# nv-tlabs/ASE

Hardware: NVIDIA H100
Metric: training env-steps/sec HumanoidAMPGetup 4096 envs/GPU (higher is better)
Workload: dtype f32 (3xFP16 scaled hi/lo tensor-core products, fp32 accumulate)

## Files before the change

ase_b200/csrc/gemm_tc.cu:

```cuda
#include <cuda.h>
#include <cuda_fp16.h>
#include <vector>
#include <unordered_map>
#include <string.h>
#include <stdlib.h>
#include "common.cuh"
#include "kernels.h"
#include "tc_common.cuh"

namespace ase {


template <bool H>
__device__ __forceinline__ void epilogue_rows(const TcEpi& e, const float* cs, int cs_ld, float* s_colsum, int row0, int nrows, int BNT, int m0, int n0, int lane) {
  const bool vec_ok = ((e.ldc & 3) == 0) && ((reinterpret_cast<uintptr_t>(e.C) & 15) == 0) &&
                      (!e.mask_mode || e.mask_bits || (((e.ldm & 3) == 0) && ((reinterpret_cast<uintptr_t>(e.mask_src) & 15) == 0)));
  const bool add_bias = e.bias && (!e.accumulate || blockIdx.z == 0);
  const uintptr_t pal = H ? 7 : 15;
  const bool pvec = e.Chi && ((e.ldp & 3) == 0) && ((reinterpret_cast<uintptr_t>(e.Chi) & pal) == 0) && ((reinterpret_cast<uintptr_t>(e.Clo) & pal) == 0);
  const float cscale = (H && e.Chi && e.c_scale) ? *e.c_scale : 1.0f;
  const bool use_bits = e.mask_mode == 1 && e.mask_bits != nullptr;
  const int nib_shift = 4 * (lane & 7);
  float amax = 0.0f;
#pragma unroll 1
  for (int cc = lane * 4; cc < ((BNT + 127) & ~127); cc += 128) {
    const int n = n0 + cc;
    const int rem = (cc < BNT) ? e.N - n : 0;
    const bool full = rem >= 4;
    const int nvalid = full ? 4 : (rem > 0 ? rem : 0);
    float bv[4] = {0.0f, 0.0f, 0.0f, 0.0f};
    if (add_bias) for (int j = 0; j < nvalid; ++j) bv[j] = e.bias[n + j];
    float cs4[4] = {0.0f, 0.0f, 0.0f, 0.0f};
#pragma unroll 4
    for (int r = 0; r < nrows; ++r) {
      const int row = row0 + r, m = m0 + row;
      if (m >= e.M) break;
      const float4 t = (cc < BNT) ? lds128(cs + row * cs_ld + cc) : make_float4(0.0f, 0.0f, 0.0f, 0.0f);
      float x[4] = {t.x + bv[0], t.y + bv[1], t.z + bv[2], t.w + bv[3]};
      float* cp = e.C + (int64_t)m * e.ldc + n;
      if (e.accumulate) {
        if (vec_ok && full) asm volatile("red.global.add.v4.f32 [%0], {%1, %2, %3, %4};" ::"l"(cp), "f"(x[0]), "f"(x[1]), "f"(x[2]), "f"(x[3]) : "memory");
        else for (int j = 0; j < nvalid; ++j) atomicAdd(cp + j, x[j]);
        continue;
      }
      if (e.act == 1) { for (int j = 0; j < 4; ++j) x[j] = fmaxf(x[j], 0.0f); }
      else if (e.act == 2) { for (int j = 0; j < 4; ++j) x[j] = tanhf(x[j]); }
      if (e.relu_bits) {
        uint32_t w = 0;
#pragma unroll
        for (int j = 0; j < 4; ++j) w |= (j < nvalid && x[j] > 0.0f) ? (1u << j) : 0u;
        w <<= nib_shift;
        w |= __shfl_xor_sync(0xffffffffu, w, 1); w |= __shfl_xor_sync(0xffffffffu, w, 2); w |= __shfl_xor_sync(0xffffffffu, w, 4);
        if ((lane & 7) == 0 && nvalid > 0) e.relu_bits[(int64_t)m * e.ldrb + (n >> 5)] = w;
      }
      if (use_bits) {
        const uint32_t w = (nvalid > 0 && !(e.debug & 16)) ? e.mask_bits[(int64_t)m * e.ldmb + (n >> 5)] >> nib_shift : 0xFu;
#pragma unroll
        for (int j = 0; j < 4; ++j) x[j] = ((w >> j) & 1u) ? x[j] : 0.0f;
      } else if (e.mask_mode && !(e.debug & 16) && nvalid > 0) {
        const float* mp = e.mask_src + (int64_t)m * e.ldm + n;
        float mv[4] = {0.0f, 0.0f, 0.0f, 0.0f};
        if (vec_ok && full) { const float4 q = *reinterpret_cast<const float4*>(mp); mv[0] = q.x; mv[1] = q.y; mv[2] = q.z; mv[3] = q.w; }
        else for (int j = 0; j < nvalid; ++j) mv[j] = mp[j];
        if (e.mask_mode == 1) { for (int j = 0; j < 4; ++j) x[j] = (mv[j] > 0.0f) ? x[j] : 0.0f; }
        else { for (int j = 0; j < 4; ++j) x[j] *= (1.0f - mv[j] * mv[j]); }
      }
      if (e.skip_c || (e.debug & 128)) {}
      else if (vec_ok && full) *reinterpret_cast<float4*>(cp) = make_float4(x[0], x[1], x[2], x[3]);
      else for (int j = 0; j < nvalid; ++j) cp[j] = x[j];
#pragma unroll
      for (int j = 0; j < 4; ++j) { cs4[j] += x[j]; if (j < nvalid) amax = fmaxf(amax, fabsf(x[j])); }
      if (e.Chi && !(e.debug & 32) && nvalid > 0) {
        if (!H) {
          float h[4], l[4];
#pragma unroll
          for (int j = 0; j < 4; ++j) split_tf32(x[j], h[j], l[j]);
          float* hp = (float*)e.Chi + (int64_t)m * e.ldp + n; float* lp = (float*)e.Clo + (int64_t)m * e.ldp + n;
          if (pvec && full) { *reinterpret_cast<float4*>(hp) = make_float4(h[0], h[1], h[2], h[3]); *reinterpret_cast<float4*>(lp) = make_float4(l[0], l[1], l[2], l[3]); }
          else for (int j = 0; j < nvalid; ++j) { hp[j] = h[j]; lp[j] = l[j]; }
        } else {
          uint2 hv, lv;
          split_f16x2(x[0] * cscale, x[1] * cscale, hv.x, lv.x); split_f16x2(x[2] * cscale, x[3] * cscale, hv.y, lv.y);
          __half* hp = (__half*)e.Chi + (int64_t)m * e.ldp + n; __half* lp = (__half*)e.Clo + (int64_t)m * e.ldp + n;
          if (pvec && full) { *reinterpret_cast<uint2*>(hp) = hv; *reinterpret_cast<uint2*>(lp) = lv; }
          else {
            const uint32_t hw[2] = {hv.x, hv.y}, lw[2] = {lv.x, lv.y};
            for (int j = 0; j < nvalid; ++j) {
              hp[j] = __ushort_as_half((unsigned short)(hw[j >> 1] >> (16 * (j & 1))));
              lp[j] = __ushort_as_half((unsigned short)(lw[j >> 1] >> (16 * (j & 1))));
            }
          }
        }
      }
    }
    if (e.colsum && !e.accumulate && !(e.debug & 64)) for (int j = 0; j < nvalid; ++j) atomicAdd(s_colsum + cc + j, cs4[j]);
  }
  if ((e.c_amax || (H && e.Chi && e.flag)) && !e.accumulate) report_scale_miss(amax, cscale, e.c_amax, (H && e.Chi) ? e.flag : nullptr);
}

__device__ __forceinline__ bool epilogue_frag_ok(const TcEpi& e, int m0, int n0, int bm, int bn, bool H) {
  if (e.accumulate || m0 + bm > e.M || n0 + bn > e.N) return false;
  if ((e.ldc & 3) || (reinterpret_cast<uintptr_t>(e.C) & 15)) return false;
  if (e.bias && (reinterpret_cast<uintptr_t>(e.bias) & 15)) return false;
  if (e.Chi && (!H || (e.ldp & 7) || (reinterpret_cast<uintptr_t>(e.Chi) & 15) || (reinterpret_cast<uintptr_t>(e.Clo) & 15))) return false;
  if (e.mask_mode && !(e.mask_mode == 1 && e.mask_bits) && ((e.ldm & 3) || (reinterpret_cast<uintptr_t>(e.mask_src) & 15))) return false;
  return true;
}

template <class T, int N> struct FragArr {
  T v[N];
  __device__ __forceinline__ T& operator[](int i) { return v[i]; }
  __device__ __forceinline__ const T& operator[](int i) const { return v[i]; }
};

template <bool H, int NH>
__device__ __forceinline__ void epilogue_frag(const TcEpi& e, float (&acc)[NH][64], float* s_colsum, int m0, int n0, int wg, int t) {
  constexpr int NROW = 2 * NH;
  constexpr unsigned FULL = 0xffffffffu;
  const int lane = t & 31, q = lane & 3;
  const bool odd = q & 1;
  const int cq = ((q & 1) << 3) | ((q & 2) << 1);
  const int64_t m = m0 + wg * NH * 64 + 16 * (t >> 5) + (lane >> 2);
  const int n = n0 + cq;
  const float s1 = (H && e.a_inv) ? *e.a_inv : 1.0f;
  const float s2 = e.alpha * ((H && e.b_inv) ? *e.b_inv : 1.0f);
  const float cscale = (H && e.Chi && e.c_scale) ? *e.c_scale : 1.0f;
  const bool use_bits = e.mask_mode == 1 && e.mask_bits != nullptr;
  const uint32_t* mb = use_bits ? e.mask_bits + m * e.ldmb + (n0 >> 5) : nullptr;
  float* cp = e.C + m * e.ldc + n;
  __half* hp = (H && e.Chi) ? (__half*)e.Chi + m * e.ldp + n : nullptr;
  __half* lp = (H && e.Chi) ? (__half*)e.Clo + m * e.ldp + n : nullptr;
  const float* mp = (e.mask_mode && !use_bits) ? e.mask_src + m * e.ldm + n : nullptr;
  const float* bp = e.bias ? e.bias + n : nullptr;
  FragArr<uint32_t, NROW> mw, mwn;
#pragma unroll
  for (int k = 0; k < NROW; ++k) { mw[k] = 0; mwn[k] = 0; }
  if (use_bits) {
#pragma unroll
    for (int k = 0; k < NROW; ++k) mw[k] = __ldg(mb + (64 * (k >> 1) + 8 * (k & 1)) * e.ldmb);
  }
  float amax = 0.0f;
  FragArr<uint32_t, NROW> rbw;
#pragma unroll
  for (int k = 0; k < NROW; ++k) rbw[k] = 0;
#pragma unroll 1
  for (int g = 0; g < 8; ++g) {
    const int w = g >> 1;
    if (use_bits && !(g & 1) && w < 3) {
#pragma unroll
      for (int k = 0; k < NROW; ++k) mwn[k] = __ldg(mb + (64 * (k >> 1) + 8 * (k & 1)) * e.ldmb + w + 1);
    }
    const int c = 16 * g, sh = 16 * (g & 1) + cq;
    FragArr<float, 4> bv = {{0.0f, 0.0f, 0.0f, 0.0f}};
    if (bp) { const float4 b4 = *reinterpret_cast<const float4*>(bp + c); bv[0] = b4.x; bv[1] = b4.y; bv[2] = b4.z; bv[3] = b4.w; }
    FragArr<float, 4> csum = {{0.0f, 0.0f, 0.0f, 0.0f}};
#pragma unroll
    for (int k = 0; k < NROW; ++k) {
      const int64_t ro = 64 * (k >> 1) + 8 * (k & 1);
      const float* a = acc[k >> 1] + 2 * (k & 1);
      const float r0 = __shfl_xor_sync(FULL, odd ? a[0] : a[4], 1), r1 = __shfl_xor_sync(FULL, odd ? a[1] : a[5], 1);
      FragArr<float, 4> x;
      x[0] = odd ? r0 : a[0]; x[1] = odd ? r1 : a[1]; x[2] = odd ? a[4] : r0; x[3] = odd ? a[5] : r1;
#pragma unroll
      for (int j = 0; j < 4; ++j) x[j] = __fadd_rn(__fmul_rn(s2, __fmul_rn(s1, x[j])), bv[j]);
      if (e.act == 1) {
#pragma unroll
        for (int j = 0; j < 4; ++j) x[j] = fmaxf(x[j], 0.0f);
      } else if (e.act == 2) {
#pragma unroll
        for (int j = 0; j < 4; ++j) x[j] = tanhf(x[j]);
      }
      if (e.relu_bits) {
        uint32_t nib = 0;
#pragma unroll
        for (int j = 0; j < 4; ++j) nib |= (x[j] > 0.0f) ? (1u << j) : 0u;
        rbw[k] |= nib << sh;
      }
      if (use_bits) {
#pragma unroll
        for (int j = 0; j < 4; ++j) x[j] = ((mw[k] >> (sh + j)) & 1u) ? x[j] : 0.0f;
      } else if (mp) {
        const float4 q4 = *reinterpret_cast<const float4*>(mp + ro * e.ldm + c);
        const FragArr<float, 4> mv = {{q4.x, q4.y, q4.z, q4.w}};
        if (e.mask_mode == 1) {
#pragma unroll
          for (int j = 0; j < 4; ++j) x[j] = (mv[j] > 0.0f) ? x[j] : 0.0f;
        } else {
#pragma unroll
          for (int j = 0; j < 4; ++j) x[j] *= (1.0f - mv[j] * mv[j]);
        }
      }
      if (!e.skip_c) *reinterpret_cast<float4*>(cp + ro * e.ldc + c) = make_float4(x[0], x[1], x[2], x[3]);
#pragma unroll
      for (int j = 0; j < 4; ++j) { csum[j] += x[j]; amax = fmaxf(amax, fabsf(x[j])); }
      if (H && hp) {
        uint2 hv, lv;
        split_f16x2(x[0] * cscale, x[1] * cscale, hv.x, lv.x); split_f16x2(x[2] * cscale, x[3] * cscale, hv.y, lv.y);
        *reinterpret_cast<uint2*>(hp + ro * e.ldp + c) = hv;
        *reinterpret_cast<uint2*>(lp + ro * e.ldp + c) = lv;
      }
    }
    if (e.colsum) {
#pragma unroll
      for (int j = 0; j < 4; ++j) {
        float v = csum[j];
        v += __shfl_xor_sync(FULL, v, 4); v += __shfl_xor_sync(FULL, v, 8); v += __shfl_xor_sync(FULL, v, 16);
        if (lane < 4) atomicAdd(s_colsum + c + cq + j, v);
      }
    }
    if (e.relu_bits && (g & 1)) {
      uint32_t word = 0;
#pragma unroll
      for (int k = 0; k < NROW; ++k) {
        uint32_t v = rbw[k];
        v |= __shfl_xor_sync(FULL, v, 1); v |= __shfl_xor_sync(FULL, v, 2);
        if (q == k) word = v;
        rbw[k] = 0;
      }
      if (q < NROW) e.relu_bits[(m + 64 * (q >> 1) + 8 * (q & 1)) * e.ldrb + (n0 >> 5) + w] = word;
    }
    if (g & 1) {
#pragma unroll
      for (int k = 0; k < NROW; ++k) mw[k] = mwn[k];
    }
#pragma unroll
    for (int h = 0; h < NH; ++h)
#pragma unroll
      for (int i = 0; i < 56; ++i) acc[h][i] = acc[h][i + 8];
  }
  if (e.c_amax || (H && e.Chi && e.flag)) report_scale_miss(amax, cscale, e.c_amax, (H && e.Chi) ? e.flag : nullptr);
}

template <int BM, int BN> constexpr int tc_stages() { return (200 * 1024) / (256 * (BM + BN)); }

template <int BM, int BN, int STAGES>
struct TcSmem {
  static constexpr int A_BYTES = BM * 128;
  static constexpr int B_BYTES = BN * 128;
  static constexpr int STAGE_BYTES = 2 * A_BYTES + 2 * B_BYTES;
  static constexpr int COLSUM_OFF = STAGES * STAGE_BYTES + 256;
  static constexpr int TOTAL = COLSUM_OFF + 512 + 1024 ;
  static_assert(BM * (BN + 4) * 4 <= STAGES * STAGE_BYTES, "the generic store phase's staging tile lives over the ring");
};

template <int BN, bool AMN, bool BMN, bool H>
__device__ __forceinline__ void wg_mma(float (&d)[BN / 2], uint32_t a, uint32_t b, int k, int sd) {
  const uint64_t da = tc_desc<AMN>(a, k), db = tc_desc<BMN>(b, k);
  if constexpr (H) {
    if constexpr (BN == 128) wg_f16_n128<AMN, BMN>(d, da, db, sd); else wg_f16_n64<AMN, BMN>(d, da, db, sd);
  } else {
    if constexpr (BN == 128) wg_tf32_n128(d, da, db, sd); else wg_tf32_n64(d, da, db, sd);
  }
}

template <int BM, int BN, int STAGES, bool AMN, bool BMN, bool H>
__global__ void __launch_bounds__(TC_THREADS, 1)
gemm_tc_kernel(const __grid_constant__ CUtensorMap tmAhi, const __grid_constant__ CUtensorMap tmAlo,
               const __grid_constant__ CUtensorMap tmBhi, const __grid_constant__ CUtensorMap tmBlo, const TcEpi e) {
  static_assert(H || (!AMN && !BMN), "TF32 wgmma reads K-major operands only");
  static_assert(BM == 128 || BM == 256, "tile height");
  using SM = TcSmem<BM, BN, STAGES>;
  using F = TcFmt<H>;
  constexpr int R = BN / 2;
  constexpr int NH = BM / 128;
  extern __shared__ uint8_t smem_raw[];
  uint8_t* smem = reinterpret_cast<uint8_t*>((reinterpret_cast<uintptr_t>(smem_raw) + 1023) & ~uintptr_t(1023));
  uint64_t* full = reinterpret_cast<uint64_t*>(smem + STAGES * SM::STAGE_BYTES);
  uint64_t* empty = full + STAGES;

  const int warp = threadIdx.x >> 5, lane = threadIdx.x & 31;
  const int m0 = blockIdx.y * BM, n0 = blockIdx.x * BN;
  const int kb_begin = blockIdx.z * e.kb_per_split;
  const int nkb = min(e.kb_per_split, e.kb_total - kb_begin);

  if (threadIdx.x == 0) {
    asm volatile("prefetch.tensormap [%0];" ::"l"(reinterpret_cast<uint64_t>(&tmAhi)) : "memory");
    asm volatile("prefetch.tensormap [%0];" ::"l"(reinterpret_cast<uint64_t>(&tmAlo)) : "memory");
    asm volatile("prefetch.tensormap [%0];" ::"l"(reinterpret_cast<uint64_t>(&tmBhi)) : "memory");
    asm volatile("prefetch.tensormap [%0];" ::"l"(reinterpret_cast<uint64_t>(&tmBlo)) : "memory");
    for (int s = 0; s < STAGES; ++s) { mbar_init(&full[s], 1); mbar_init(&empty[s], 2); }
    asm volatile("fence.mbarrier_init.release.cluster;" ::: "memory");
  }
  float* s_colsum = reinterpret_cast<float*>(smem + SM::COLSUM_OFF);
  if (threadIdx.x < BN) s_colsum[threadIdx.x] = 0.0f;
  __syncthreads();
  pdl_sync();

  if (warp < 4) {
    asm volatile("setmaxnreg.dec.sync.aligned.u32 40;");
    if (warp == 0 && lane == 0) {
      for (int kb = 0; kb < nkb; ++kb) {
        const int s = kb % STAGES;
        const uint32_t ph = (kb / STAGES) & 1;
        mbar_wait(&empty[s], ph ^ 1);
        mbar_expect_tx(&full[s], SM::STAGE_BYTES);
        uint8_t* st = smem + s * SM::STAGE_BYTES;
        const int k0 = (kb_begin + kb) * F::BK;
        if (!AMN) {
          tma_load_2d(st, &tmAhi, &full[s], k0, m0);
          tma_load_2d(st + SM::A_BYTES, &tmAlo, &full[s], k0, m0);
        } else {
#pragma unroll
          for (int b = 0; b < BM / F::MN_BOX; ++b) {
            tma_load_2d(st + b * F::MN_BOX_BYTES, &tmAhi, &full[s], m0 + b * F::MN_BOX, k0);
            tma_load_2d(st + SM::A_BYTES + b * F::MN_BOX_BYTES, &tmAlo, &full[s], m0 + b * F::MN_BOX, k0);
          }
        }
        if (!BMN) {
          tma_load_2d(st + 2 * SM::A_BYTES, &tmBhi, &full[s], k0, n0);
          tma_load_2d(st + 2 * SM::A_BYTES + SM::B_BYTES, &tmBlo, &full[s], k0, n0);
        } else {
#pragma unroll
          for (int b = 0; b < BN / F::MN_BOX; ++b) {
            tma_load_2d(st + 2 * SM::A_BYTES + b * F::MN_BOX_BYTES, &tmBhi, &full[s], n0 + b * F::MN_BOX, k0);
            tma_load_2d(st + 2 * SM::A_BYTES + SM::B_BYTES + b * F::MN_BOX_BYTES, &tmBlo, &full[s], n0 + b * F::MN_BOX, k0);
          }
        }
      }
    }
    return;
  }
  asm volatile("setmaxnreg.inc.sync.aligned.u32 232;");
  const int wg = (warp >> 2) - 1;
  const int t = threadIdx.x & 127;
  const bool corrections = !(e.debug & 4);
  float acc[NH][R], part[R];
#pragma unroll
  for (int h = 0; h < NH; ++h)
#pragma unroll
    for (int j = 0; j < R; ++j) acc[h][j] = 0.0f;
  for (int kb = 0; kb < nkb; ++kb) {
    const int s = kb % STAGES;
    mbar_wait(&full[s], (kb / STAGES) & 1);
    const uint32_t sa = smem_u32(smem + s * SM::STAGE_BYTES);
    const uint32_t b_hi = sa + 2 * SM::A_BYTES, b_lo = b_hi + SM::B_BYTES;
#pragma unroll
    for (int h = 0; h < NH; ++h) {
      const uint32_t a_hi = sa + (wg * NH + h) * TC_M64_BYTES, a_lo = a_hi + SM::A_BYTES;
      wg_fence();
      if (corrections) {
#pragma unroll
        for (int k = 0; k < 4; ++k) {
          wg_mma<BN, AMN, BMN, H>(part, a_lo, b_hi, k, k > 0 ? 1 : 0);
          wg_mma<BN, AMN, BMN, H>(part, a_hi, b_lo, k, 1);
        }
      }
#pragma unroll
      for (int k = 0; k < 4; ++k) wg_mma<BN, AMN, BMN, H>(part, a_hi, b_hi, k, (corrections || k > 0) ? 1 : 0);
      wg_commit();
      wg_wait<0>();
      if (h == NH - 1 && t == 0) mbar_arrive(&empty[s]);
#pragma unroll
      for (int j = 0; j < R; ++j) acc[h][j] += part[j];
    }
  }
  const int et = threadIdx.x - 128;
  bool frag = false;
  if constexpr (BN == 128) frag = epilogue_frag_ok(e, m0, n0, BM, BN, H) && !(e.debug & 256);
  if (frag) {
    if constexpr (BN == 128) { if (!(e.debug & 1)) epilogue_frag<H, NH>(e, acc, s_colsum, m0, n0, wg, t); }
  } else {
    asm volatile("bar.sync 1, 256;" ::: "memory");
    float* cs = reinterpret_cast<float*>(smem);
    constexpr int CS_LD = BN + 4;
    const float s1 = (H && e.a_inv) ? *e.a_inv : 1.0f;
    const float s2 = e.alpha * ((H && e.b_inv) ? *e.b_inv : 1.0f);
#pragma unroll
    for (int h = 0; h < NH; ++h) {
      const int row = (wg * NH + h) * 64 + 16 * (t >> 5) + ((t & 31) >> 2);
      float* c0 = cs + row * CS_LD + 2 * (t & 3);
#pragma unroll
      for (int j = 0; j < R / 4; ++j) {
        const float* a = acc[h] + 4 * j;
        asm volatile("st.shared.v2.f32 [%0], {%1, %2};" ::"r"(smem_u32(c0 + 8 * j)), "f"(s2 * (s1 * a[0])), "f"(s2 * (s1 * a[1])) : "memory");
        asm volatile("st.shared.v2.f32 [%0], {%1, %2};" ::"r"(smem_u32(c0 + 8 * CS_LD + 8 * j)), "f"(s2 * (s1 * a[2])), "f"(s2 * (s1 * a[3])) : "memory");
      }
    }
    asm volatile("bar.sync 1, 256;" ::: "memory");
    constexpr int NRW = BM / 8;
    if (!(e.debug & 1)) epilogue_rows<H>(e, cs, CS_LD, s_colsum, (warp - 4) * NRW, NRW, BN, m0, n0, lane);
  }
  if (e.colsum && !e.accumulate) {
    asm volatile("bar.sync 1, 256;" ::: "memory");
    if (et < BN && n0 + et < e.N) atomicAdd(e.colsum + n0 + et, s_colsum[et]);
  }
}


__global__ void __launch_bounds__(256)
tc_prep_kernel(const float* __restrict__ src, int64_t ld, int rows, int cols, int rows_p, int cols_p, float* __restrict__ hi,
               float* __restrict__ lo) {
  const int64_t total = (int64_t)rows_p * cols_p;
  for (int64_t i = (int64_t)blockIdx.x * blockDim.x + threadIdx.x; i < total; i += (int64_t)gridDim.x * blockDim.x) {
    const int r = (int)(i / cols_p), c = (int)(i - (int64_t)r * cols_p);
    float h = 0.0f, l = 0.0f;
    if (r < rows && c < cols) split_tf32(src[(int64_t)r * ld + c], h, l);
    hi[i] = h; lo[i] = l;
  }
}

__global__ void __launch_bounds__(256)
tc_prep_t_kernel(const float* __restrict__ src, int64_t ld, int rows, int cols, int cols_p, float* __restrict__ hi,
                 float* __restrict__ lo) {
  __shared__ float tile[32][33];
  const int r0 = blockIdx.x * 32, c0 = blockIdx.y * 32, tx = threadIdx.x;
  for (int j = threadIdx.y; j < 32; j += 8) {
    const int c = c0 + j, r = r0 + tx;
    tile[j][tx] = (r < rows && c < cols) ? src[(int64_t)c * ld + r] : 0.0f;
  }
  __syncthreads();
  for (int j = threadIdx.y; j < 32; j += 8) {
    const int64_t o = (int64_t)(r0 + j) * cols_p + c0 + tx;
    float h, l;
    split_tf32(tile[tx][j], h, l);
    hi[o] = h; lo[o] = l;
  }
}

template <int N>
__global__ void __launch_bounds__(256)
tc_amax_kernel(const TcPrepList<N> l) {
  const TcPrepItem it = l.item[blockIdx.y];
  const int64_t total = (int64_t)it.rows * it.cols;
  float m = 0.0f;
  if (it.cols == it.ld) {
    for (int64_t i = (int64_t)blockIdx.x * blockDim.x + threadIdx.x; i < total; i += (int64_t)gridDim.x * blockDim.x) m = fmaxf(m, fabsf(it.src[i]));
  } else {
    for (int64_t i = (int64_t)blockIdx.x * blockDim.x + threadIdx.x; i < total; i += (int64_t)gridDim.x * blockDim.x) {
      const int r = (int)(i / it.cols), c = (int)(i - (int64_t)r * it.cols);
      m = fmaxf(m, fabsf(it.src[(int64_t)r * it.ld + c]));
    }
  }
  report_scale_miss(m, 1.0f, it.amax, nullptr);
}

template <int N>
__global__ void __launch_bounds__(256)
tc_split_h_kernel(const TcPrepList<N> l, int exact, int top, unsigned* __restrict__ flag) {
  const TcPrepItem it = l.item[blockIdx.y];
  float s;
  if (exact) {
    s = scale_from_amax(__uint_as_float(*it.amax), top);
    if (blockIdx.x == 0 && threadIdx.x == 0) { it.scale[0] = s; it.scale[1] = 1.0f / s; }
  } else s = it.scale[0];
  if (it.scale_copy && blockIdx.x == 0 && threadIdx.x == 0) { it.scale_copy[0] = s; it.scale_copy[1] = (s != 0.0f) ? 1.0f / s : 0.0f; }
  __half* hi = (__half*)it.hi; __half* lo = (__half*)it.lo;
  const int c4n = it.ldp >> 2;
  const int64_t total = (int64_t)it.rows_p * c4n;
  const bool vec = ((it.ld & 3) == 0) && ((reinterpret_cast<uintptr_t>(it.src) & 15) == 0);
  float m = 0.0f;
  for (int64_t i = (int64_t)blockIdx.x * blockDim.x + threadIdx.x; i < total; i += (int64_t)gridDim.x * blockDim.x) {
    const int r = (int)(i / c4n), c = (int)(i - (int64_t)r * c4n) * 4;
    float x[4] = {0.0f, 0.0f, 0.0f, 0.0f};
    if (r < it.rows) {
      const float* sp = it.src + (int64_t)r * it.ld + c;
      if (vec && c + 4 <= it.cols) { const float4 t = *reinterpret_cast<const float4*>(sp); x[0] = t.x; x[1] = t.y; x[2] = t.z; x[3] = t.w; }
      else for (int j = 0; j < 4; ++j) if (c + j < it.cols) x[j] = sp[j];
    }
#pragma unroll
    for (int j = 0; j < 4; ++j) m = fmaxf(m, fabsf(x[j]));
    uint2 hv, lv;
    split_f16x2(x[0] * s, x[1] * s, hv.x, lv.x); split_f16x2(x[2] * s, x[3] * s, hv.y, lv.y);
    *reinterpret_cast<uint2*>(hi + (int64_t)r * it.ldp + c) = hv;
    *reinterpret_cast<uint2*>(lo + (int64_t)r * it.ldp + c) = lv;
  }
  if (!exact) report_scale_miss(m, s, it.amax, flag);
}
// ... 58 lines not shown
  cuuint32_t box[2] = {half ? 64u : 32u, (cuuint32_t)box_rows};
  cuuint32_t estr[2] = {1, 1};
  if (mn_major && !half) { set_error("wgmma GEMM: TF32 planes cannot be read MN-major"); return ASE_ERR_INVALID; }
  CUresult r = enc(tm, half ? CU_TENSOR_MAP_DATA_TYPE_FLOAT16 : CU_TENSOR_MAP_DATA_TYPE_FLOAT32, 2, (void*)base, gdim, gstr, box, estr,
                   CU_TENSOR_MAP_INTERLEAVE_NONE, CU_TENSOR_MAP_SWIZZLE_128B,
                   CU_TENSOR_MAP_L2_PROMOTION_L2_128B, CU_TENSOR_MAP_FLOAT_OOB_FILL_NONE);
  if (r != CUDA_SUCCESS) { set_error("cuTensorMapEncodeTiled(%d x %d, ld %lld, box %d) failed with CUresult %d", rows, cols, (long long)ld, box_rows, (int)r); return ASE_ERR_CUDA; }
  if (c.size() > 8192) c.clear();
  c.emplace(k, *tm);
  return ASE_OK;
}

static inline int pad_to(int x, int m) { return (x + m - 1) / m * m; }

constexpr int64_t TC_WS_HEAD = 1024;
constexpr int TC_MPAD = 256;
struct TcWsSlots { int64_t a, b; };
static TcWsSlots tc_ws_slots(int M, int N, int K) {
  const int64_t Mp = pad_to(M, TC_MPAD), Np = pad_to(N, 128), Kw = pad_to(K, TC_KPAD);
  return {align_up(Mp * Kw * 4, 1024), align_up(Np * Kw * 4, 1024)};
}
int64_t gemm_tc_workspace_bytes(int M, int N, int K) {
  const TcWsSlots s = tc_ws_slots(M, N, K);
  return TC_WS_HEAD + 2 * s.a + 2 * s.b;
}

int gemm_tc_check_workspace(const AseGemmParams& p) {
  if (!p.workspace || p.workspace_bytes < gemm_tc_workspace_bytes(p.M, p.N, p.K)) {
    set_error("wgmma GEMM %dx%dx%d: workspace %lld bytes < required %lld", p.M, p.N, p.K, (long long)p.workspace_bytes,
              (long long)gemm_tc_workspace_bytes(p.M, p.N, p.K));
    return ASE_ERR_WORKSPACE;
  }
  if (reinterpret_cast<uintptr_t>(p.workspace) & 1023) { set_error("wgmma GEMM: workspace must be 1024-byte aligned"); return ASE_ERR_WORKSPACE; }
  return ASE_OK;
}

static int prep_operand(const float* src, int64_t ld, int trans, int rows, int K, int rows_p, int Kp, float* hi, float* lo, cudaStream_t st) {
  if (trans) {
    tc_prep_t_kernel<<<dim3(rows_p / 32, Kp / 32), dim3(32, 8), 0, st>>>(src, ld, rows, K, Kp, hi, lo);
  } else {
    const int64_t total = (int64_t)rows_p * Kp;
    tc_prep_kernel<<<(int)imin64((total + 255) / 256, NUM_SMS * 16), 256, 0, st>>>(src, ld, rows, K, rows_p, Kp, hi, lo);
  }
  ASE_LAUNCH_OK();
  return ASE_OK;
}

static int materialize_h(const TcPrepItem& it, bool scale_known, bool max_known, unsigned* flag, int top, cudaStream_t st) {
  const TcPrepList<1> l{{it}};
  if (!scale_known && !max_known) {
    const int64_t total = (int64_t)it.rows * it.cols;
    tc_amax_kernel<1><<<(int)imin64((total + 1023) / 1024, NUM_SMS * 8), 256, 0, st>>>(l);
    ASE_LAUNCH_OK();
  }
  const int64_t total = (int64_t)it.rows_p * (it.ldp / 4);
  tc_split_h_kernel<1><<<(int)imin64((total + 255) / 256, NUM_SMS * 16), 256, 0, st>>>(l, scale_known ? 0 : 1, top, flag);
  ASE_LAUNCH_OK();
  return ASE_OK;
}

struct TcProfile {
  bool on = false;
  std::vector<cudaEvent_t> ev;
  size_t used = 0;
  double flops = 0.0;
};
static TcProfile g_prof;

static void prof_mark(cudaStream_t st) {
  if (g_prof.used == g_prof.ev.size()) {
    cudaEvent_t e;
    if (cudaEventCreate(&e) != cudaSuccess) { g_prof.on = false; return; }
    g_prof.ev.push_back(e);
  }
  cudaEventRecord(g_prof.ev[g_prof.used++], st);
}

static int tc_pdl() {
  static int v = -1;
  if (v < 0) { const char* d = getenv("ASE_TC_PDL"); v = d ? (atoi(d) != 0) : 1; }
  return v;
}

template <int BM, int BN, bool AMN, bool BMN, bool H>
static int launch_tc(const CUtensorMap& ah, const CUtensorMap& al, const CUtensorMap& bh, const CUtensorMap& bl, const TcEpi& e,
                     int splits, cudaStream_t st) {
  constexpr int STAGES = tc_stages<BM, BN>();
  using SM = TcSmem<BM, BN, STAGES>;
  static bool attr_set = false;
  if (!attr_set) {
    ASE_CUDA_OK(cudaFuncSetAttribute(gemm_tc_kernel<BM, BN, STAGES, AMN, BMN, H>, cudaFuncAttributeMaxDynamicSharedMemorySize, SM::TOTAL));
    attr_set = true;
  }
  dim3 grid(ceil_div(e.N, BN), ceil_div(e.M, BM), splits);
  const bool prof = g_prof.on;
  if (prof) prof_mark(st);
  cudaLaunchConfig_t cfg = {};
  cfg.gridDim = grid; cfg.blockDim = dim3(TC_THREADS); cfg.dynamicSmemBytes = SM::TOTAL; cfg.stream = st;
  cudaLaunchAttribute attr[1];
  attr[0].id = cudaLaunchAttributeProgrammaticStreamSerialization;
  attr[0].val.programmaticStreamSerializationAllowed = tc_pdl();
  cfg.attrs = attr; cfg.numAttrs = 1;
  ASE_CUDA_OK(cudaLaunchKernelEx(&cfg, gemm_tc_kernel<BM, BN, STAGES, AMN, BMN, H>, ah, al, bh, bl, e));
  if (prof) { prof_mark(st); g_prof.flops += 2.0 * (double)e.M * (double)e.N * (double)e.K; }
  ASE_LAUNCH_OK();
  return ASE_OK;
}

template <int BM, int BN, bool H>
static int launch_tc_major(bool amn, bool bmn, const CUtensorMap& ah, const CUtensorMap& al, const CUtensorMap& bh, const CUtensorMap& bl,
                           const TcEpi& e, int splits, cudaStream_t st) {
  if constexpr (!H) {
    if (amn || bmn) { set_error("wgmma GEMM: TF32 operand planes must be K-major"); return ASE_ERR_INVALID; }
    return launch_tc<BM, BN, false, false, false>(ah, al, bh, bl, e, splits, st);
  } else {
    if (!amn && !bmn) return launch_tc<BM, BN, false, false, true>(ah, al, bh, bl, e, splits, st);
    if (!amn && bmn) return launch_tc<BM, BN, false, true, true>(ah, al, bh, bl, e, splits, st);
    if (amn && !bmn) return launch_tc<BM, BN, true, false, true>(ah, al, bh, bl, e, splits, st);
    return launch_tc<BM, BN, true, true, true>(ah, al, bh, bl, e, splits, st);
  }
}

static int tc_debug() {
  static int v = -1;
  if (v < 0) { const char* d = getenv("ASE_TC_DEBUG"); v = d ? atoi(d) : 0; }
  return v;
}

constexpr double TC_CTA_FIXED = 1.0, TC_CTA_STORE = 1.0;
TcPlan gemm_tc_plan(int M, int N, int K, int accumulate, int split_k, int sms, bool f16) {
  TcPlan best{128, N > 64 ? 128 : 64, 1};
  const int kb_total = ceil_div(K, f16 ? TcFmt<true>::BK : TcFmt<false>::BK);
  int smin = 1, smax = 1;
  if (accumulate && split_k > 1) smin = smax = min(split_k, kb_total);
  else if (accumulate && split_k < 0) smax = max(1, min(64, kb_total / 4));
  const int bm_max = (tc_debug() & 512) ? 128 : 256;
  double best_cost = 1e300;
  for (int bm = 128; bm <= bm_max; bm *= 2) {
    for (int s = smin; s <= smax; ++s) {
      const int kbs = ceil_div(kb_total, s), splits = ceil_div(kb_total, kbs);
      const int64_t ctas = (int64_t)ceil_div(M, bm) * ceil_div(N, best.bn) * splits;
      const double area = (double)bm * best.bn / (128.0 * 128.0);
      const double cost = (double)ceil_div(ctas, (int64_t)sms) * (TC_CTA_FIXED + (kbs + TC_CTA_STORE) * area) * (1.0 + 0.03 * splits);
      if (cost < best_cost - 1e-9) { best_cost = cost; best.bm = bm; best.splits = splits; }
    }
  }
  return best;
}

PlaneBuf* PlaneRegistry::find(const float* p) {
  for (int i = 0; i < n; ++i)
    if (p >= b[i].base && p < b[i].base + b[i].capacity) return &b[i];
  return nullptr;
}
void PlaneRegistry::add(const float* base, int64_t capacity, float* hi, float* lo, int64_t plane_capacity) {
  if (n >= MAX) return;
  PlaneBuf& x = b[n++];
  x.base = base; x.capacity = capacity; x.hi = hi; x.lo = lo; x.plane_capacity = plane_capacity;
  x.ld = 0; x.rows = x.cols = 0; x.ldp = 0; x.scale_ptr = nullptr; x.drop();
}
PlaneBuf* PlaneRegistry::declare(const float* base, int64_t ld, int rows, int cols) {
  PlaneBuf* x = find(base);
  if (!x || x->base != base) return nullptr;
  x->drop();
  const int64_t ldp = f16 ? (cols + 7) / 8 * 8 : (cols + 3) / 4 * 4;
  if ((int64_t)rows * ldp > (f16 ? 2 : 1) * x->plane_capacity) return nullptr;
  x->ld = ld; x->rows = rows; x->cols = cols; x->ldp = ldp; x->valid = true;
  if (f16) { x->is_static = true; x->scale_ptr = static_scale; }
  return x;
}
void* PlaneRegistry::plane(const PlaneBuf* x, bool lo, int64_t r0, int64_t c0) const {
  float* p = lo ? x->lo : x->hi;
  const int64_t off = r0 * x->ldp + c0;
  return f16 ? (void*)((__half*)p + off) : (void*)(p + off);
}
void PlaneRegistry::invalidate(const float* p) { if (PlaneBuf* x = find(p)) x->drop(); }
void PlaneRegistry::invalidate_range(const float* lo_, const float* hi_) {
  for (int i = 0; i < n; ++i) if (b[i].base >= lo_ && b[i].base < hi_) b[i].drop();
}
int PlaneRegistry::begin_call(cudaStream_t st, int base) {
  call_base = base; gemm_index = 0;
  if (!f16) return ASE_OK;
  if (reset_pending) {
    ASE_CUDA_OK(cudaMemsetAsync(amax, 0, (size_t)SITES * 12, st));
    reset_pending = false;
  }
  for (int i = 0; i < SITES; ++i) { if (touched[i]) { known[i] = true; touched[i] = false; } }
  for (int i = 0; i < n; ++i) {
    b[i].amax_site = -1;
    if (b[i].valid && !b[i].is_static && b[i].scale_ptr >= scale && b[i].scale_ptr < scale + 2 * SITES) b[i].valid = false;
    if (b[i].is_static) { b[i].valid = false; b[i].is_static = false; }
  }
  tc_site_update_kernel<<<ceil_div(SITES, 256), 256, 0, st>>>(amax, scale, SITES, static_scale, STATIC_SCALE, flag);
  ASE_LAUNCH_OK();
  return ASE_OK;
}

int PlaneRegistry::prep_weights(const float* const* src, const int* rows, const int* cols, int count, cudaStream_t st) {
  if (!f16 || count <= 0) return ASE_OK;
  TcPrepBatch batch; int nb = 0; bool all_known = true;
  for (int i = 0; i < count && nb < TcPrepBatch::MAX; ++i) {
    PlaneBuf* x = find(src[i]);
// ... 104 lines not shown
      }
    } else {
      ASE_CUDA_OK(cudaMemsetAsync(ws, 0, 2 * sizeof(unsigned), st));
      t_amax[0] = (unsigned*)ws; t_amax[1] = (unsigned*)ws + 1; t_scale[0] = (float*)(ws + 16); t_scale[1] = (float*)(ws + 32);
    }
  }
  unsigned* oflag = (H && reg) ? reg->flag : nullptr;
  char* wsp = ws + TC_WS_HEAD;
  const TcWsSlots slots = tc_ws_slots(p.M, p.N, p.K);
  if (va.ok) {
    if ((rc = encode_cached(&ah, va.hi, a_rows, a_cols, va.ldp, p.a_trans ? BK : a_box, p.a_trans != 0, H)) ||
        (rc = encode_cached(&al, va.lo, a_rows, a_cols, va.ldp, p.a_trans ? BK : a_box, p.a_trans != 0, H))) return rc;
  } else {
    float* Ahi = (float*)wsp; float* Alo = (float*)(wsp + slots.a);
    if (!H) { if ((rc = prep_operand(p.A, p.lda, p.a_trans, p.M, p.K, Mp, Kp, Ahi, Alo, st))) return rc; }
    else {
      const TcPrepItem it{p.A, p.lda, a_rows, a_cols, p.a_trans ? Kp : Mp, p.a_trans ? Mp : Kp, Ahi, Alo, t_amax[0], t_scale[0], nullptr};
      if ((rc = materialize_h(it, t_pred[0], false, oflag, reg ? TOP_SITE : TOP_EXACT, st))) return rc;
      va.scale = t_scale[0];
    }
    if (!p.a_trans || !H) { if ((rc = encode_cached(&ah, Ahi, Mp, Kp, Kp, a_box, false, H)) || (rc = encode_cached(&al, Alo, Mp, Kp, Kp, a_box, false, H))) return rc; }
    else            { if ((rc = encode_cached(&ah, Ahi, Kp, Mp, Mp, BK, true, H)) || (rc = encode_cached(&al, Alo, Kp, Mp, Mp, BK, true, H))) return rc; }
  }
  if (vb.ok) {
    if ((rc = encode_cached(&bh, vb.hi, b_rows, b_cols, vb.ldp, p.b_trans ? BK : BN, p.b_trans != 0, H)) ||
        (rc = encode_cached(&bl, vb.lo, b_rows, b_cols, vb.ldp, p.b_trans ? BK : BN, p.b_trans != 0, H))) return rc;
  } else {
    char* wb = wsp + 2 * slots.a;
    float* Bhi = (float*)wb; float* Blo = (float*)(wb + slots.b);
    if (!H) { if ((rc = prep_operand(p.B, p.ldb, p.b_trans, p.N, p.K, Np, Kp, Bhi, Blo, st))) return rc; }
    else {
      const TcPrepItem it{p.B, p.ldb, b_rows, b_cols, p.b_trans ? Kp : Np, p.b_trans ? Np : Kp, Bhi, Blo, t_amax[1], t_scale[1], nullptr};
      if ((rc = materialize_h(it, t_pred[1], false, oflag, reg ? TOP_SITE : TOP_EXACT, st))) return rc;
      vb.scale = t_scale[1];
    }
    if (!p.b_trans || !H) { if ((rc = encode_cached(&bh, Bhi, Np, Kp, Kp, BN, false, H)) || (rc = encode_cached(&bl, Blo, Np, Kp, Kp, BN, false, H))) return rc; }
    else            { if ((rc = encode_cached(&bh, Bhi, Kp, Np, Np, BK, true, H)) || (rc = encode_cached(&bl, Blo, Kp, Np, Np, BK, true, H))) return rc; }
  }
  TcEpi e;
  e.C = p.C; e.ldc = p.ldc; e.M = p.M; e.N = p.N; e.K = p.K; e.alpha = p.alpha; e.bias = p.bias; e.act = p.act;
  e.mask_src = p.mask_src; e.ldm = p.ldm; e.mask_mode = p.mask_src ? p.mask_mode : 0; e.accumulate = p.accumulate;
  e.Chi = e.Clo = nullptr; e.ldp = 0; e.colsum = p.colsum_out;
  e.a_inv = (H && va.scale) ? va.scale + 1 : nullptr; e.b_inv = (H && vb.scale) ? vb.scale + 1 : nullptr;
  e.c_scale = nullptr; e.c_amax = nullptr; e.flag = nullptr;
  e.relu_bits = p.relu_bits_out; e.ldrb = p.ldrb; e.mask_bits = (e.mask_mode == 1) ? p.mask_bits : nullptr; e.ldmb = p.ldmb; e.skip_c = 0;
  if (reg && !H) {
    if (PlaneBuf* x = reg->find(p.C)) {
      if (p.accumulate) x->valid = false;
      else if (p.C == x->base && (int64_t)p.M * pad_to(p.N, 4) <= x->plane_capacity && !(x->valid && x->ld == p.ldc && (x->rows > p.M || x->cols > p.N))) {
        x->ld = p.ldc; x->rows = p.M; x->cols = p.N; x->ldp = pad_to(p.N, 4); x->valid = true;
        e.Chi = x->hi; e.Clo = x->lo; e.ldp = x->ldp;
      } else if (x->valid && x->ld == p.ldc) {
        const int64_t off = p.C - x->base, r0 = off / x->ld, c0 = off - r0 * x->ld;
        if (r0 + p.M <= x->rows && c0 + p.N <= x->cols) { e.Chi = x->hi + r0 * x->ldp + c0; e.Clo = x->lo + r0 * x->ldp + c0; e.ldp = x->ldp; }
        else x->valid = false;
      } else x->valid = false;
    }
  } else if (reg && H) {
    if (PlaneBuf* x = reg->find(p.C)) {
      if (x->fp32_stale && p.accumulate) { set_error("wgmma GEMM: accumulating into a planes-only tensor"); return ASE_ERR_INVALID; }
      x->fp32_stale = false;
      const bool full = !p.accumulate && p.C == x->base && (int64_t)p.M * pad_to(p.N, 8) <= 2 * x->plane_capacity && (int64_t)(p.M - 1) * p.ldc + p.N <= x->capacity &&
                        !(x->valid && x->is_static && x->ld == p.ldc && (x->rows > p.M || x->cols > p.N));
      if (full) {
        x->ld = p.ldc; x->rows = p.M; x->cols = p.N; x->ldp = pad_to(p.N, 8); x->is_static = false;
        reg->touched[site_c] = true; e.c_amax = reg->amax + site_c;
        if (reg->known[site_c]) {
          x->valid = true; x->amax_site = -1; x->scale_ptr = reg->scale + 2 * site_c;
          e.Chi = x->hi; e.Clo = x->lo; e.ldp = x->ldp; e.c_scale = x->scale_ptr; e.flag = reg->flag;
          if (p.c_planes_only) { e.skip_c = 1; x->fp32_stale = true; }
        } else { x->valid = false; x->amax_site = site_c; }
      } else if (!p.accumulate && x->valid && x->is_static && x->ld == p.ldc && p.act == 2 && !p.mask_src) {
        const int64_t off = p.C - x->base, r0 = off / x->ld, c0 = off - r0 * x->ld;
        if (r0 + p.M <= x->rows && c0 + p.N <= x->cols) { e.Chi = reg->plane(x, false, r0, c0); e.Clo = reg->plane(x, true, r0, c0); e.ldp = x->ldp; e.c_scale = x->scale_ptr; e.flag = reg->flag; }
        else x->drop();
      } else x->drop();
    }
  }
  e.kb_total = ceil_div(p.K, BK);
  e.debug = tc_debug();
  e.kb_per_split = ceil_div(e.kb_total, plan.splits);
  const int splits = ceil_div(e.kb_total, e.kb_per_split);
  const bool amn = H && p.a_trans, bmn = H && p.b_trans;
  if (H) {
    if (plan.bm == 256) return BN == 128 ? launch_tc_major<256, 128, true>(amn, bmn, ah, al, bh, bl, e, splits, st)
                                         : launch_tc_major<256, 64, true>(amn, bmn, ah, al, bh, bl, e, splits, st);
    return BN == 128 ? launch_tc_major<128, 128, true>(amn, bmn, ah, al, bh, bl, e, splits, st)
                     : launch_tc_major<128, 64, true>(amn, bmn, ah, al, bh, bl, e, splits, st);
  }
  if (plan.bm == 256) return BN == 128 ? launch_tc_major<256, 128, false>(amn, bmn, ah, al, bh, bl, e, splits, st)
                                       : launch_tc_major<256, 64, false>(amn, bmn, ah, al, bh, bl, e, splits, st);
  return BN == 128 ? launch_tc_major<128, 128, false>(amn, bmn, ah, al, bh, bl, e, splits, st)
                   : launch_tc_major<128, 64, false>(amn, bmn, ah, al, bh, bl, e, splits, st);
}

}

extern "C" int ase_gemm_tc_plan(int M, int N, int K, int accumulate, int split_k, int backend, int* tile_m, int* tile_n, int* splits) {
  using namespace ase;
  if (M < 1 || N < 1 || K < 1 || (backend != 1 && backend != 2)) { set_error("ase_gemm_tc_plan: bad shape or backend"); return ASE_ERR_INVALID; }
  const TcPlan p = gemm_tc_plan(M, N, K, accumulate, split_k, NUM_SMS, backend == 2);
  if (tile_m) *tile_m = p.bm;
  if (tile_n) *tile_n = p.bn;
  if (splits) *splits = p.splits;
  return ASE_OK;
}

extern "C" int ase_gemm_tc_profile(int enable) {
  ase::g_prof.on = enable != 0;
  ase::g_prof.used = 0;
  ase::g_prof.flops = 0.0;
  return ASE_OK;
}

extern "C" int ase_gemm_tc_profile_read(double* total_ms, int64_t* launches, double* flops) {
  using namespace ase;
  double tot = 0.0;
  const size_t n = g_prof.used / 2;
  for (size_t i = 0; i < n; ++i) {
    float ms = 0.0f;
    ASE_CUDA_OK(cudaEventSynchronize(g_prof.ev[2 * i + 1]));
    ASE_CUDA_OK(cudaEventElapsedTime(&ms, g_prof.ev[2 * i], g_prof.ev[2 * i + 1]));
    tot += ms;
  }
  if (total_ms) *total_ms = tot;
  if (launches) *launches = (int64_t)n;
  if (flops) *flops = g_prof.flops;
  return ASE_OK;
}
```

Baseline: 411,500.

## Add persistent tile-loop variant of FP16 wgmma GEMM for evenly divisible shapes

Adds a persistent mode to the TMA/wgmma GEMM kernel. It launches at most one CTA per SM, and each CTA loops over output tiles, so the producer warp keeps prefetching the next tile's operands while consumers run the previous tile's epilogue. It is used for FP16 3-pass GEMMs with BN=128, shapes divisible by the tile, and frag-epilogue eligibility. Column sums are double-buffered in shared memory to allow this. It costs an extra kernel instantiation and ignores the split-K plan on this path, which could hurt shapes that relied on split-K parallelism.

```diff
diff --git a/ase_b200/csrc/gemm_tc.cu b/ase_b200/csrc/gemm_tc.cu
--- a/ase_b200/csrc/gemm_tc.cu
+++ b/ase_b200/csrc/gemm_tc.cu
@@ -98,7 +98,7 @@
   if ((e.c_amax || (H && e.Chi && e.flag)) && !e.accumulate) report_scale_miss(amax, cscale, e.c_amax, (H && e.Chi) ? e.flag : nullptr);
 }
 
-__device__ __forceinline__ bool epilogue_frag_ok(const TcEpi& e, int m0, int n0, int bm, int bn, bool H) {
+__host__ __device__ __forceinline__ bool epilogue_frag_ok(const TcEpi& e, int m0, int n0, int bm, int bn, bool H) {
   if (e.accumulate || m0 + bm > e.M || n0 + bn > e.N) return false;
   if ((e.ldc & 3) || (reinterpret_cast<uintptr_t>(e.C) & 15)) return false;
   if (e.bias && (reinterpret_cast<uintptr_t>(e.bias) & 15)) return false;
@@ -239,7 +239,7 @@
   static constexpr int B_BYTES = BN * 128;
   static constexpr int STAGE_BYTES = 2 * A_BYTES + 2 * B_BYTES;
   static constexpr int COLSUM_OFF = STAGES * STAGE_BYTES + 256;
-  static constexpr int TOTAL = COLSUM_OFF + 512 + 1024 ;
+  static constexpr int TOTAL = COLSUM_OFF + 2 * 512 + 1024 ;
   static_assert(BM * (BN + 4) * 4 <= STAGES * STAGE_BYTES, "the generic store phase's staging tile lives over the ring");
 };
 
@@ -253,12 +253,13 @@
   }
 }
 
-template <int BM, int BN, int STAGES, bool AMN, bool BMN, bool H>
+template <int BM, int BN, int STAGES, bool AMN, bool BMN, bool H, bool PERSIST>
 __global__ void __launch_bounds__(TC_THREADS, 1)
 gemm_tc_kernel(const __grid_constant__ CUtensorMap tmAhi, const __grid_constant__ CUtensorMap tmAlo,
                const __grid_constant__ CUtensorMap tmBhi, const __grid_constant__ CUtensorMap tmBlo, const TcEpi e) {
   static_assert(H || (!AMN && !BMN), "TF32 wgmma reads K-major operands only");
   static_assert(BM == 128 || BM == 256, "tile height");
+  static_assert(!PERSIST || (H && BN == 128), "the persistent kernel stores every tile from the fragments");
   using SM = TcSmem<BM, BN, STAGES>;
   using F = TcFmt<H>;
   constexpr int R = BN / 2;
@@ -269,9 +270,13 @@
   uint64_t* empty = full + STAGES;
 
   const int warp = threadIdx.x >> 5, lane = threadIdx.x & 31;
-  const int m0 = blockIdx.y * BM, n0 = blockIdx.x * BN;
-  const int kb_begin = blockIdx.z * e.kb_per_split;
-  const int nkb = min(e.kb_per_split, e.kb_total - kb_begin);
+  const int kb_begin = PERSIST ? 0 : blockIdx.z * e.kb_per_split;
+  const int nkb = PERSIST ? e.kb_total : min(e.kb_per_split, e.kb_total - kb_begin);
+  const int tiles_n = PERSIST ? e.N / BN : 1;
+  const int ntiles = PERSIST ? (e.M / BM) * tiles_n : 1;
+  const int tile0 = PERSIST ? (int)blockIdx.x : 0, tile_step = PERSIST ? (int)gridDim.x : 1;
+  auto tile_m0 = [&](int tile) { return PERSIST ? (tile / tiles_n) * BM : (int)blockIdx.y * BM; };
+  auto tile_n0 = [&](int tile) { return PERSIST ? (tile % tiles_n) * BN : (int)blockIdx.x * BN; };
 
   if (threadIdx.x == 0) {
     asm volatile("prefetch.tensormap [%0];" ::"l"(reinterpret_cast<uint64_t>(&tmAhi)) : "memory");
@@ -282,38 +287,42 @@
     asm volatile("fence.mbarrier_init.release.cluster;" ::: "memory");
   }
   float* s_colsum = reinterpret_cast<float*>(smem + SM::COLSUM_OFF);
-  if (threadIdx.x < BN) s_colsum[threadIdx.x] = 0.0f;
+  if (threadIdx.x < 2 * BN) s_colsum[threadIdx.x] = 0.0f;
   __syncthreads();
   pdl_sync();
 
   if (warp < 4) {
     asm volatile("setmaxnreg.dec.sync.aligned.u32 40;");
     if (warp == 0 && lane == 0) {
-      for (int kb = 0; kb < nkb; ++kb) {
-        const int s = kb % STAGES;
-        const uint32_t ph = (kb / STAGES) & 1;
-        mbar_wait(&empty[s], ph ^ 1);
-        mbar_expect_tx(&full[s], SM::STAGE_BYTES);
-        uint8_t* st = smem + s * SM::STAGE_BYTES;
-        const int k0 = (kb_begin + kb) * F::BK;
-        if (!AMN) {
-          tma_load_2d(st, &tmAhi, &full[s], k0, m0);
-          tma_load_2d(st + SM::A_BYTES, &tmAlo, &full[s], k0, m0);
-        } else {
-#pragma unroll
-          for (int b = 0; b < BM / F::MN_BOX; ++b) {
-            tma_load_2d(st + b * F::MN_BOX_BYTES, &tmAhi, &full[s], m0 + b * F::MN_BOX, k0);
-            tma_load_2d(st + SM::A_BYTES + b * F::MN_BOX_BYTES, &tmAlo, &full[s], m0 + b * F::MN_BOX, k0);
+      int it = 0;
+      for (int tile = tile0; tile < ntiles; tile += tile_step) {
+        const int m0 = tile_m0(tile), n0 = tile_n0(tile);
+        for (int kb = 0; kb < nkb; ++kb, ++it) {
+          const int s = it % STAGES;
+          const uint32_t ph = (it / STAGES) & 1;
+          mbar_wait(&empty[s], ph ^ 1);
+          mbar_expect_tx(&full[s], SM::STAGE_BYTES);
+          uint8_t* st = smem + s * SM::STAGE_BYTES;
+          const int k0 = (kb_begin + kb) * F::BK;
+          if (!AMN) {
+            tma_load_2d(st, &tmAhi, &full[s], k0, m0);
+            tma_load_2d(st + SM::A_BYTES, &tmAlo, &full[s], k0, m0);
+          } else {
+#pragma unroll
+            for (int b = 0; b < BM / F::MN_BOX; ++b) {
+              tma_load_2d(st + b * F::MN_BOX_BYTES, &tmAhi, &full[s], m0 + b * F::MN_BOX, k0);
+              tma_load_2d(st + SM::A_BYTES + b * F::MN_BOX_BYTES, &tmAlo, &full[s], m0 + b * F::MN_BOX, k0);
+            }
           }
-        }
-        if (!BMN) {
-          tma_load_2d(st + 2 * SM::A_BYTES, &tmBhi, &full[s], k0, n0);
-          tma_load_2d(st + 2 * SM::A_BYTES + SM::B_BYTES, &tmBlo, &full[s], k0, n0);
-        } else {
-#pragma unroll
-          for (int b = 0; b < BN / F::MN_BOX; ++b) {
-            tma_load_2d(st + 2 * SM::A_BYTES + b * F::MN_BOX_BYTES, &tmBhi, &full[s], n0 + b * F::MN_BOX, k0);
-            tma_load_2d(st + 2 * SM::A_BYTES + SM::B_BYTES + b * F::MN_BOX_BYTES, &tmBlo, &full[s], n0 + b * F::MN_BOX, k0);
+          if (!BMN) {
+            tma_load_2d(st + 2 * SM::A_BYTES, &tmBhi, &full[s], k0, n0);
+            tma_load_2d(st + 2 * SM::A_BYTES + SM::B_BYTES, &tmBlo, &full[s], k0, n0);
+          } else {
+#pragma unroll
+            for (int b = 0; b < BN / F::MN_BOX; ++b) {
+              tma_load_2d(st + 2 * SM::A_BYTES + b * F::MN_BOX_BYTES, &tmBhi, &full[s], n0 + b * F::MN_BOX, k0);
+              tma_load_2d(st + 2 * SM::A_BYTES + SM::B_BYTES + b * F::MN_BOX_BYTES, &tmBlo, &full[s], n0 + b * F::MN_BOX, k0);
+            }
           }
         }
       }
@@ -323,66 +332,78 @@
   asm volatile("setmaxnreg.inc.sync.aligned.u32 232;");
   const int wg = (warp >> 2) - 1;
   const int t = threadIdx.x & 127;
+  const int et = threadIdx.x - 128;
   const bool corrections = !(e.debug & 4);
-  float acc[NH][R], part[R];
-#pragma unroll
-  for (int h = 0; h < NH; ++h)
-#pragma unroll
-    for (int j = 0; j < R; ++j) acc[h][j] = 0.0f;
-  for (int kb = 0; kb < nkb; ++kb) {
-    const int s = kb % STAGES;
-    mbar_wait(&full[s], (kb / STAGES) & 1);
-    const uint32_t sa = smem_u32(smem + s * SM::STAGE_BYTES);
-    const uint32_t b_hi = sa + 2 * SM::A_BYTES, b_lo = b_hi + SM::B_BYTES;
-#pragma unroll
-    for (int h = 0; h < NH; ++h) {
-      const uint32_t a_hi = sa + (wg * NH + h) * TC_M64_BYTES, a_lo = a_hi + SM::A_BYTES;
-      wg_fence();
-      if (corrections) {
-#pragma unroll
-        for (int k = 0; k < 4; ++k) {
-          wg_mma<BN, AMN, BMN, H>(part, a_lo, b_hi, k, k > 0 ? 1 : 0);
-          wg_mma<BN, AMN, BMN, H>(part, a_hi, b_lo, k, 1);
+#pragma unroll 1
+  for (int tile = tile0; tile < ntiles; tile += tile_step) {
+    const int ti = tile / tile_step;
+    float acc[NH][R], part[R];
+#pragma unroll
+    for (int h = 0; h < NH; ++h)
+#pragma unroll
+      for (int j = 0; j < R; ++j) acc[h][j] = 0.0f;
+    if constexpr (PERSIST) {
+#pragma unroll
+      for (int j = 0; j < R; ++j) part[j] = 0.0f;
+    }
+    for (int kb = 0; kb < nkb; ++kb) {
+      const int it = ti * nkb + kb;
+      const int s = it % STAGES;
+      mbar_wait(&full[s], (it / STAGES) & 1);
+      const uint32_t sa = smem_u32(smem + s * SM::STAGE_BYTES);
+      const uint32_t b_hi = sa + 2 * SM::A_BYTES, b_lo = b_hi + SM::B_BYTES;
+#pragma unroll
+      for (int h = 0; h < NH; ++h) {
+        const uint32_t a_hi = sa + (wg * NH + h) * TC_M64_BYTES, a_lo = a_hi + SM::A_BYTES;
+        wg_fence();
+        if (corrections) {
+#pragma unroll
+          for (int k = 0; k < 4; ++k) {
+            wg_mma<BN, AMN, BMN, H>(part, a_lo, b_hi, k, k > 0 ? 1 : 0);
+            wg_mma<BN, AMN, BMN, H>(part, a_hi, b_lo, k, 1);
+          }
         }
-      }
-#pragma unroll
-      for (int k = 0; k < 4; ++k) wg_mma<BN, AMN, BMN, H>(part, a_hi, b_hi, k, (corrections || k > 0) ? 1 : 0);
-      wg_commit();
-      wg_wait<0>();
-      if (h == NH - 1 && t == 0) mbar_arrive(&empty[s]);
-#pragma unroll
-      for (int j = 0; j < R; ++j) acc[h][j] += part[j];
-    }
-  }
-  const int et = threadIdx.x - 128;
-  bool frag = false;
-  if constexpr (BN == 128) frag = epilogue_frag_ok(e, m0, n0, BM, BN, H) && !(e.debug & 256);
-  if (frag) {
-    if constexpr (BN == 128) { if (!(e.debug & 1)) epilogue_frag<H, NH>(e, acc, s_colsum, m0, n0, wg, t); }
-  } else {
-    asm volatile("bar.sync 1, 256;" ::: "memory");
-    float* cs = reinterpret_cast<float*>(smem);
-    constexpr int CS_LD = BN + 4;
-    const float s1 = (H && e.a_inv) ? *e.a_inv : 1.0f;
-    const float s2 = e.alpha * ((H && e.b_inv) ? *e.b_inv : 1.0f);
-#pragma unroll
-    for (int h = 0; h < NH; ++h) {
-      const int row = (wg * NH + h) * 64 + 16 * (t >> 5) + ((t & 31) >> 2);
-      float* c0 = cs + row * CS_LD + 2 * (t & 3);
-#pragma unroll
-      for (int j = 0; j < R / 4; ++j) {
-        const float* a = acc[h] + 4 * j;
-        asm volatile("st.shared.v2.f32 [%0], {%1, %2};" ::"r"(smem_u32(c0 + 8 * j)), "f"(s2 * (s1 * a[0])), "f"(s2 * (s1 * a[1])) : "memory");
-        asm volatile("st.shared.v2.f32 [%0], {%1, %2};" ::"r"(smem_u32(c0 + 8 * CS_LD + 8 * j)), "f"(s2 * (s1 * a[2])), "f"(s2 * (s1 * a[3])) : "memory");
-      }
-    }
-    asm volatile("bar.sync 1, 256;" ::: "memory");
-    constexpr int NRW = BM / 8;
-    if (!(e.debug & 1)) epilogue_rows<H>(e, cs, CS_LD, s_colsum, (warp - 4) * NRW, NRW, BN, m0, n0, lane);
-  }
-  if (e.colsum && !e.accumulate) {
-    asm volatile("bar.sync 1, 256;" ::: "memory");
-    if (et < BN && n0 + et < e.N) atomicAdd(e.colsum + n0 + et, s_colsum[et]);
+#pragma unroll
+        for (int k = 0; k < 4; ++k) wg_mma<BN, AMN, BMN, H>(part, a_hi, b_hi, k, (corrections || k > 0) ? 1 : 0);
+        wg_commit();
+        wg_wait<0>();
+        if (h == NH - 1 && t == 0) mbar_arrive(&empty[s]);
+#pragma unroll
+        for (int j = 0; j < R; ++j) acc[h][j] += part[j];
+      }
+    }
+    const int m0 = tile_m0(tile), n0 = tile_n0(tile);
+    float* cs_slot = s_colsum + (PERSIST ? (ti & 1) * BN : 0);
+    bool frag = PERSIST;
+    if constexpr (BN == 128 && !PERSIST) frag = epilogue_frag_ok(e, m0, n0, BM, BN, H) && !(e.debug & 256);
+    if (frag) {
+      if constexpr (BN == 128) { if (!(e.debug & 1)) epilogue_frag<H, NH>(e, acc, cs_slot, m0, n0, wg, t); }
+    } else if constexpr (!PERSIST) {
+      asm volatile("bar.sync 1, 256;" ::: "memory");
+      float* cs = reinterpret_cast<float*>(smem);
+      constexpr int CS_LD = BN + 4;
+      const float s1 = (H && e.a_inv) ? *e.a_inv : 1.0f;
+      const float s2 = e.alpha * ((H && e.b_inv) ? *e.b_inv : 1.0f);
+#pragma unroll
+      for (int h = 0; h < NH; ++h) {
+        const int row = (wg * NH + h) * 64 + 16 * (t >> 5) + ((t & 31) >> 2);
+        float* c0 = cs + row * CS_LD + 2 * (t & 3);
+#pragma unroll
+        for (int j = 0; j < R / 4; ++j) {
+          const float* a = acc[h] + 4 * j;
+          asm volatile("st.shared.v2.f32 [%0], {%1, %2};" ::"r"(smem_u32(c0 + 8 * j)), "f"(s2 * (s1 * a[0])), "f"(s2 * (s1 * a[1])) : "memory");
+          asm volatile("st.shared.v2.f32 [%0], {%1, %2};" ::"r"(smem_u32(c0 + 8 * CS_LD + 8 * j)), "f"(s2 * (s1 * a[2])), "f"(s2 * (s1 * a[3])) : "memory");
+        }
+      }
+      asm volatile("bar.sync 1, 256;" ::: "memory");
+      constexpr int NRW = BM / 8;
+      if (!(e.debug & 1)) epilogue_rows<H>(e, cs, CS_LD, s_colsum, (warp - 4) * NRW, NRW, BN, m0, n0, lane);
+    }
+    if (e.colsum && !e.accumulate) {
+      asm volatile("bar.sync 1, 256;" ::: "memory");
+      if (et < BN && n0 + et < e.N) atomicAdd(e.colsum + n0 + et, cs_slot[et]);
+      if (PERSIST && et < BN) cs_slot[et] = 0.0f;
+    }
   }
 }
 
@@ -607,17 +628,17 @@
   return v;
 }
 
-template <int BM, int BN, bool AMN, bool BMN, bool H>
+template <int BM, int BN, bool AMN, bool BMN, bool H, bool PERSIST>
 static int launch_tc(const CUtensorMap& ah, const CUtensorMap& al, const CUtensorMap& bh, const CUtensorMap& bl, const TcEpi& e,
                      int splits, cudaStream_t st) {
   constexpr int STAGES = tc_stages<BM, BN>();
   using SM = TcSmem<BM, BN, STAGES>;
   static bool attr_set = false;
   if (!attr_set) {
-    ASE_CUDA_OK(cudaFuncSetAttribute(gemm_tc_kernel<BM, BN, STAGES, AMN, BMN, H>, cudaFuncAttributeMaxDynamicSharedMemorySize, SM::TOTAL));
+    ASE_CUDA_OK(cudaFuncSetAttribute(gemm_tc_kernel<BM, BN, STAGES, AMN, BMN, H, PERSIST>, cudaFuncAttributeMaxDynamicSharedMemorySize, SM::TOTAL));
     attr_set = true;
   }
-  dim3 grid(ceil_div(e.N, BN), ceil_div(e.M, BM), splits);
+  const dim3 grid = PERSIST ? dim3(min((e.M / BM) * (e.N / BN), NUM_SMS)) : dim3(ceil_div(e.N, BN), ceil_div(e.M, BM), splits);
   const bool prof = g_prof.on;
   if (prof) prof_mark(st);
   cudaLaunchConfig_t cfg = {};
@@ -626,23 +647,23 @@
   attr[0].id = cudaLaunchAttributeProgrammaticStreamSerialization;
   attr[0].val.programmaticStreamSerializationAllowed = tc_pdl();
   cfg.attrs = attr; cfg.numAttrs = 1;
-  ASE_CUDA_OK(cudaLaunchKernelEx(&cfg, gemm_tc_kernel<BM, BN, STAGES, AMN, BMN, H>, ah, al, bh, bl, e));
+  ASE_CUDA_OK(cudaLaunchKernelEx(&cfg, gemm_tc_kernel<BM, BN, STAGES, AMN, BMN, H, PERSIST>, ah, al, bh, bl, e));
   if (prof) { prof_mark(st); g_prof.flops += 2.0 * (double)e.M * (double)e.N * (double)e.K; }
   ASE_LAUNCH_OK();
   return ASE_OK;
 }
 
-template <int BM, int BN, bool H>
+template <int BM, int BN, bool H, bool PERSIST = false>
 static int launch_tc_major(bool amn, bool bmn, const CUtensorMap& ah, const CUtensorMap& al, const CUtensorMap& bh, const CUtensorMap& bl,
                            const TcEpi& e, int splits, cudaStream_t st) {
   if constexpr (!H) {
     if (amn || bmn) { set_error("wgmma GEMM: TF32 operand planes must be K-major"); return ASE_ERR_INVALID; }
-    return launch_tc<BM, BN, false, false, false>(ah, al, bh, bl, e, splits, st);
+    return launch_tc<BM, BN, false, false, false, false>(ah, al, bh, bl, e, splits, st);
   } else {
-    if (!amn && !bmn) return launch_tc<BM, BN, false, false, true>(ah, al, bh, bl, e, splits, st);
-    if (!amn && bmn) return launch_tc<BM, BN, false, true, true>(ah, al, bh, bl, e, splits, st);
-    if (amn && !bmn) return launch_tc<BM, BN, true, false, true>(ah, al, bh, bl, e, splits, st);
-    return launch_tc<BM, BN, true, true, true>(ah, al, bh, bl, e, splits, st);
+    if (!amn && !bmn) return launch_tc<BM, BN, false, false, true, PERSIST>(ah, al, bh, bl, e, splits, st);
+    if (!amn && bmn) return launch_tc<BM, BN, false, true, true, PERSIST>(ah, al, bh, bl, e, splits, st);
+    if (amn && !bmn) return launch_tc<BM, BN, true, false, true, PERSIST>(ah, al, bh, bl, e, splits, st);
+    return launch_tc<BM, BN, true, true, true, PERSIST>(ah, al, bh, bl, e, splits, st);
   }
 }
 
@@ -913,6 +934,10 @@
   e.kb_per_split = ceil_div(e.kb_total, plan.splits);
   const int splits = ceil_div(e.kb_total, e.kb_per_split);
   const bool amn = H && p.a_trans, bmn = H && p.b_trans;
+  const bool persist = H && BN == 128 && !(e.debug & (256 | 1024)) && p.M % plan.bm == 0 && p.N % BN == 0 &&
+                       epilogue_frag_ok(e, 0, 0, plan.bm, BN, H);
+  if (persist) return plan.bm == 256 ? launch_tc_major<256, 128, true, true>(amn, bmn, ah, al, bh, bl, e, splits, st)
+                                     : launch_tc_major<128, 128, true, true>(amn, bmn, ah, al, bh, bl, e, splits, st);
   if (H) {
     if (plan.bm == 256) return BN == 128 ? launch_tc_major<256, 128, true>(amn, bmn, ah, al, bh, bl, e, splits, st)
                                          : launch_tc_major<256, 64, true>(amn, bmn, ah, al, bh, bl, e, splits, st);
```

New measurement: 430,500, median of 6. 1.05x the previous value.
